# lich0031/AIDE

Measured on AMD Instinct MI355X. Metric: training images/sec FuseUNet 256x256x2 bs=4/GPU, higher is better.
Workload: dtype f32; 1 GPU; c2 fuseunet fwd+loss+bwd+Adam(amsgrad), 256x256 2-modal, bs=4/GPU, fp32; global_batch=4, parallelism=dp1

## Files before the change

aide_amd/csrc/conv3x3_winograd.hip:

```cpp
#include "common.h"

namespace {

struct WinoArgs {
    const float* x;
    const float* u;
    const float* bias;
    float* y;
    long x_bs, y_bs, split_stride;
    int N, Cin, H, W, Cout;
    int tiles_w, tiles_h, n_co_tiles, splitk, chunks_total, accumulate;
};

constexpr int WCK = 8;
constexpr int WTCO = 64;
constexpr int RROWS = 18, RRS = 24;
constexpr int RCS = RROWS * RRS + 8;
constexpr int RAWL = WCK * RCS;
constexpr int VL = 16 * 64 * WCK;
constexpr int UL = 16 * WTCO * WCK;
constexpr int WBUF = RAWL + VL + UL;

__global__ __launch_bounds__(256, 1) void conv3x3_wino_kernel(const WinoArgs a) {
    extern __shared__ __attribute__((aligned(16))) float lds[];
    const int tid = threadIdx.x, lane = tid & 63, wid = tid >> 6;
    const int half = lane >> 5, j = lane & 31;
    const int wave_m = wid >> 1, wave_n = wid & 1;

    int b = xcd_remap(blockIdx.x, gridDim.x);
    const int co_tile = b % a.n_co_tiles; b /= a.n_co_tiles;
    const int split = b % a.splitk;       b /= a.splitk;
    const int tw = b % a.tiles_w;         b /= a.tiles_w;
    const int th = b % a.tiles_h;
    const int n = b / a.tiles_h;
    const int h0 = th * 16, w0 = tw * 16, co0 = co_tile * WTCO;
    const int HW = a.H * a.W;

    const int cps = (a.chunks_total + a.splitk - 1) / a.splitk;
    const int c_begin = split * cps;
    const int c_end = min(c_begin + cps, a.chunks_total);

    constexpr int NRB = 3, NRC = 2, NU = UL / 4 / 256;
    unsigned offB[NRB], ldsB[NRB], offC[NRC], ldsC[NRC], offU[NU];
#pragma unroll
    for (int e = 0; e < NRB; ++e) {
        int q = tid + e * 256;
        if (q >= WCK * RROWS * 4) q -= 256;
        const int c = q / (RROWS * 4), rem = q - c * (RROWS * 4), r = rem / 4, s4 = rem - r * 4;
        const int ih = h0 - 1 + r, iw = w0 + 4 * s4;
        const bool ok = ih >= 0 && ih < a.H && iw < a.W;
        offB[e] = ok ? (unsigned)(c * HW + r * a.W + 1 + 4 * s4) * 4u : BUF_OOB;
        ldsB[e] = (unsigned)(c * RCS + r * RRS + 4 + 4 * s4);
    }
#pragma unroll
    for (int e = 0; e < NRC; ++e) {
        int q = tid + e * 256;
        if (q >= WCK * RROWS * 2) q -= 256;
        const int c = q / (RROWS * 2), rem = q - c * (RROWS * 2), r = rem / 2, side = rem - r * 2;
        const int ih = h0 - 1 + r, iw = side ? w0 + 16 : w0 - 1;
        const bool ok = ih >= 0 && ih < a.H && iw >= 0 && iw < a.W;
        offC[e] = ok ? (unsigned)(c * HW + r * a.W + (side ? 17 : 0)) * 4u : BUF_OOB;
        ldsC[e] = (unsigned)(c * RCS + r * RRS + (side ? 20 : 3));
    }
#pragma unroll
    for (int v = 0; v < NU; ++v) {
        const int f = tid + v * 256;
        const int pp = f / (WTCO * WCK / 4), w4 = f - pp * (WTCO * WCK / 4);
        offU[v] = (unsigned)(pp * a.Cout * WCK + w4 * 4) * 4u;
    }
    const __amdgpu_buffer_rsrc_t xrs =
        make_rsrc(a.x + (long)n * a.x_bs + (long)h0 * a.W + w0 - (a.W + 1));
    const __amdgpu_buffer_rsrc_t urs = make_rsrc(a.u + (long)co0 * WCK);

    f32x4 rb[NRB], ru[NU];
    float rc[NRC];
    auto fetch_raw = [&](int l, int chunk) {
        const unsigned xs = (unsigned)(min(chunk, c_end - 1) * WCK) * (unsigned)HW * 4u;
        if (l < NRB) rb[l] = buf_load_f32x4(xrs, offB[l], xs);
        else rc[l - NRB] = buf_load_f32(xrs, offC[l - NRB], xs);
    };
    auto put_raw = [&](int l, float* raw) {
        if (l < NRB) *reinterpret_cast<f32x4*>(raw + ldsB[l]) = rb[l];
        else raw[ldsC[l - NRB]] = rc[l - NRB];
    };
    auto fetch_u = [&](int v, int chunk) {
        const unsigned us = (unsigned)min(chunk, c_end - 1) * 16u * (unsigned)a.Cout * (unsigned)WCK * 4u;
        ru[v] = buf_load_f32x4(urs, offU[v], us);
    };
    auto put_u = [&](int v, float* ubuf) { *reinterpret_cast<f32x4*>(ubuf + (tid + v * 256) * 4) = ru[v]; };

    f32x2 td[16], to[16];
    const int xci = lane & 7, xtj = lane >> 3;
    const int xr_off = xci * RCS + 4 * wid * RRS + 3 + 2 * xtj;
    const int xw_off = (2 * wid * 8 + xtj) * WCK + xci;
    auto xf_read = [&](int i, const float* raw) {
        td[i].x = raw[xr_off + (i / 4) * RRS + (i % 4)];
        td[i].y = raw[xr_off + (2 + i / 4) * RRS + (i % 4)];
    };
    auto xf_math = [&]() {
        f32x2 tt[16];
#pragma unroll
        for (int c = 0; c < 4; ++c) {
            tt[c] = td[c] - td[8 + c]; tt[4 + c] = td[4 + c] + td[8 + c];
            tt[8 + c] = td[8 + c] - td[4 + c]; tt[12 + c] = td[4 + c] - td[12 + c];
        }
#pragma unroll
        for (int r = 0; r < 4; ++r) {
            to[r * 4] = tt[r * 4] - tt[r * 4 + 2]; to[r * 4 + 1] = tt[r * 4 + 1] + tt[r * 4 + 2];
            to[r * 4 + 2] = tt[r * 4 + 2] - tt[r * 4 + 1]; to[r * 4 + 3] = tt[r * 4 + 1] - tt[r * 4 + 3];
        }
    };
    auto xf_store = [&](int o, float* vbuf) {
        vbuf[o * 64 * WCK + xw_off] = to[o].x;
        vbuf[o * 64 * WCK + xw_off + 8 * WCK] = to[o].y;
    };

    f32x16 acc[16];
#pragma unroll
    for (int p = 0; p < 16; ++p)
#pragma unroll
        for (int r = 0; r < 16; ++r) acc[p][r] = 0.0f;

    float* set0 = lds;
    float* set1 = lds + WBUF;
#pragma unroll
    for (int l = 0; l < NRB + NRC; ++l) fetch_raw(l, c_begin);
#pragma unroll
    for (int v = 0; v < NU; ++v) fetch_u(v, c_begin);
#pragma unroll
    for (int l = 0; l < NRB + NRC; ++l) put_raw(l, set0);
#pragma unroll
    for (int v = 0; v < NU; ++v) put_u(v, set0 + RAWL + VL);
#pragma unroll
    for (int l = 0; l < NRB + NRC; ++l) fetch_raw(l, c_begin + 1);
    __syncthreads();
#pragma unroll
    for (int i = 0; i < 16; ++i) xf_read(i, set0);
    xf_math();
#pragma unroll
    for (int o = 0; o < 16; ++o) xf_store(o, set0 + RAWL);
#pragma unroll
    for (int l = 0; l < NRB + NRC; ++l) put_raw(l, set1);
    __syncthreads();

    int cur = 0;
    for (int chunk = c_begin; chunk < c_end; ++chunk) {
        float* sc = cur ? set1 : set0;
        float* sn = cur ? set0 : set1;
        const float* la = sc + RAWL + VL + (wave_m * 32 + j) * WCK + half * 4;
        const float* lb = sc + RAWL + (wave_n * 32 + j) * WCK + half * 4;
        constexpr int STEPS = 16 * (WCK / 2);
        f32x4 a0A, b0A, a1A, b1A, a0B, b0B, a1B, b1B;
        auto frag = [&](int p, f32x4& af, f32x4& bf) {
            af = *reinterpret_cast<const f32x4*>(la + p * WTCO * WCK);
            bf = *reinterpret_cast<const f32x4*>(lb + p * 64 * WCK);
        };
        auto slot = [&](int st, const f32x4& a0c, const f32x4& b0c, const f32x4& a1c, const f32x4& b1c,
                        f32x4& a0n, f32x4& b0n, f32x4& a1n, f32x4& b1n) {
            const int g2 = st >> 3, k = st & 7, q = k >> 1;
            if (k == 0 && g2 + 1 < 8) { frag(2 * g2 + 2, a0n, b0n); frag(2 * g2 + 3, a1n, b1n); }
            if (k & 1) acc[2 * g2 + 1] = __builtin_amdgcn_mfma_f32_32x32x2f32(a1c[q], b1c[q], acc[2 * g2 + 1], 0, 0, 0);
            else acc[2 * g2] = __builtin_amdgcn_mfma_f32_32x32x2f32(a0c[q], b0c[q], acc[2 * g2], 0, 0, 0);
            if (st < NU) fetch_u(st, chunk + 1);
            else if (st < NU + NRB + NRC) fetch_raw(st - NU, chunk + 2);
            if (st >= 4 && st < 20) xf_read(st - 4, sn);
            if (st == 24) xf_math();
            if (st >= 26 && st < 42) xf_store(st - 26, sn + RAWL);
            if (st >= 44 && st < 44 + NU) put_u(st - 44, sn + RAWL + VL);
            if (st >= 52 && st < 52 + NRB + NRC) put_raw(st - 52, sc);
            __builtin_amdgcn_sched_barrier(0);
        };
        frag(0, a0A, b0A); frag(1, a1A, b1A);
#pragma unroll
        for (int st = 0; st < STEPS; st += 16) {
#pragma unroll
            for (int k = 0; k < 8; ++k) slot(st + k, a0A, b0A, a1A, b1A, a0B, b0B, a1B, b1B);
#pragma unroll
            for (int k = 0; k < 8; ++k) slot(st + 8 + k, a0B, b0B, a1B, b1B, a0A, b0A, a1A, b1A);
        }
        __syncthreads();
        cur ^= 1;
    }

    float* yn = a.y + (long)split * a.split_stride + (long)n * a.y_bs;
    const bool add_bias = (a.bias != nullptr) && (split == 0);
    const int tile = wave_n * 32 + j, ti = tile >> 3, tj = tile & 7;
    const int oh = h0 + 2 * ti, ow = w0 + 2 * tj;
    const bool pok = oh < a.H && ow < a.W;
    float bvs[16];
#pragma unroll
    for (int r = 0; r < 16; ++r) {
        const int co = co0 + wave_m * 32 + (r & 3) + 8 * (r >> 2) + 4 * half;
        bvs[r] = (add_bias && pok && co < a.Cout) ? a.bias[co] : 0.f;
    }
#pragma unroll
    for (int r4 = 0; r4 < 16; r4 += 4) {
        float2 olds[4][2];
#pragma unroll
        for (int q = 0; q < 4; ++q) {
            const int co = co0 + wave_m * 32 + q + 8 * (r4 >> 2) + 4 * half;
#pragma unroll
            for (int i = 0; i < 2; ++i)
                olds[q][i] = (a.accumulate && pok && co < a.Cout)
                                 ? *reinterpret_cast<const float2*>(yn + (long)co * HW + (long)(oh + i) * a.W + ow) : make_float2(0.f, 0.f);
        }
#pragma unroll
        for (int q = 0; q < 4; ++q) {
            const int r = r4 + q;
            const int co = co0 + wave_m * 32 + (r & 3) + 8 * (r >> 2) + 4 * half;
            float s[2][4];
#pragma unroll
            for (int c = 0; c < 4; ++c) {
                const float m0 = acc[c][r], m1 = acc[4 + c][r], m2 = acc[8 + c][r], m3 = acc[12 + c][r];
                s[0][c] = m0 + m1 + m2;
                s[1][c] = m1 - m2 - m3;
            }
            if (pok && co < a.Cout) {
                const float bv = bvs[r];
#pragma unroll
                for (int i = 0; i < 2; ++i) {
                    float2 o;
                    o.x = s[i][0] + s[i][1] + s[i][2] + bv;
                    o.y = s[i][1] - s[i][2] - s[i][3] + bv;
                    float2* p = reinterpret_cast<float2*>(yn + (long)co * HW + (long)(oh + i) * a.W + ow);
                    o.x += olds[q][i].x; o.y += olds[q][i].y;
                    *p = o;
                }
            }
        }
    }
}

__global__ void wino_splitk_reduce_kernel(const float* __restrict__ slabs, long split_stride, int splitk,
                                          float* __restrict__ y, long y_bs, int C, int HW,
                                          const float* __restrict__ bias, int accumulate, long total) {
    for (long i = (long)blockIdx.x * blockDim.x + threadIdx.x; i < total;
         i += (long)gridDim.x * blockDim.x) {
        const long chw = (long)C * HW;
        const long n = i / chw, rem = i - n * chw;
        float v = slabs[i];
        for (int s = 1; s < splitk; ++s) v += slabs[(long)s * split_stride + i];
        if (bias) v += bias[rem / HW];
        float* p = y + n * y_bs + rem;
        if (accumulate) v += *p;
        *p = v;
    }
}
__global__ __launch_bounds__(256) void wino_splitk_reduce4_kernel(const float* __restrict__ slabs, long split_stride, int splitk,
                                                                  float* __restrict__ y, long y_bs, int C, int HW,
                                                                  const float* __restrict__ bias, int accumulate, long total4) {
    const long i = (long)blockIdx.x * blockDim.x + threadIdx.x;
    if (i >= total4) return;
    const long chw4 = (long)C * HW / 4;
    const long n = i / chw4, rem = (i - n * chw4) * 4;
    const float* sp = slabs + i * 4;
    f32x4 v = *reinterpret_cast<const f32x4*>(sp);
    int s = 1;
    for (; s + 4 <= splitk; s += 4) {
        const f32x4 t0 = *reinterpret_cast<const f32x4*>(sp + (long)s * split_stride);
        const f32x4 t1 = *reinterpret_cast<const f32x4*>(sp + (long)(s + 1) * split_stride);
        const f32x4 t2 = *reinterpret_cast<const f32x4*>(sp + (long)(s + 2) * split_stride);
        const f32x4 t3 = *reinterpret_cast<const f32x4*>(sp + (long)(s + 3) * split_stride);
        v = (((v + t0) + t1) + t2) + t3;
    }
    for (; s < splitk; ++s) v += *reinterpret_cast<const f32x4*>(sp + (long)s * split_stride);
    if (bias) v += bias[rem / HW];
    float* p = y + n * y_bs + rem;
    if (accumulate) v += *reinterpret_cast<const f32x4*>(p);
    *reinterpret_cast<f32x4*>(p) = v;
}

struct WinoPackDesc {
    const float* w; float* uf; float* ud;
    int Co, Ci, ci_pad, co_pad;
    long block_start;
};

__device__ __forceinline__ void wino_g(const float g[9], float u[16]) {
    float t[12];
#pragma unroll
    for (int c = 0; c < 3; ++c) {
        const float g0 = g[c], g1 = g[3 + c], g2 = g[6 + c];
        t[c] = g0; t[3 + c] = 0.5f * (g0 + g1 + g2); t[6 + c] = 0.5f * (g0 - g1 + g2); t[9 + c] = g2;
    }
#pragma unroll
    for (int r = 0; r < 4; ++r) {
        const float a0 = t[r * 3], a1 = t[r * 3 + 1], a2 = t[r * 3 + 2];
        u[r * 4] = a0; u[r * 4 + 1] = 0.5f * (a0 + a1 + a2); u[r * 4 + 2] = 0.5f * (a0 - a1 + a2); u[r * 4 + 3] = a2;
    }
}

constexpr int WP_T = 32;
__global__ __launch_bounds__(256) void wino_pack_multi_kernel(const WinoPackDesc* __restrict__ descs, int n) {
    __shared__ __attribute__((aligned(16))) float ot[16 * 256];
    const long blk = blockIdx.x;
    int lo = 0, hi = n - 1;
    while (lo < hi) {
        const int mid = (lo + hi + 1) >> 1;
        if (descs[mid].block_start <= blk) lo = mid; else hi = mid - 1;
    }
    const WinoPackDesc d = descs[lo];
    const int tid = threadIdx.x;
    const int tiles_ci = (d.Ci + WP_T - 1) / WP_T;
    const int tb = (int)(blk - d.block_start);
    const int co0 = (tb / tiles_ci) * WP_T, ci0 = (tb % tiles_ci) * WP_T;
    const int nci = min(WP_T, d.Ci - ci0);
    float g[9], u[16];
    const int lo3 = tid & 7, hi5 = tid >> 3;
    for (int grp = 0; grp < 8; ++grp) {
        const bool fwd = grp < 4;
        const int q = grp & 3;
        float* dst = fwd ? d.uf : d.ud;
        if (dst == nullptr) continue;
        const int co = fwd ? hi5 : 8 * q + lo3, ci = fwd ? 8 * q + lo3 : hi5;
        const bool live = fwd ? (ci0 + 8 * q < d.ci_pad) : (co0 + 8 * q < d.co_pad);
        if (!live) continue;
        {
            const bool in = co0 + co < d.Co && ci < nci;
            const float* wp = d.w + ((long)(co0 + co) * d.Ci + ci0 + ci) * 9;
#pragma unroll
            for (int t = 0; t < 9; ++t) g[t] = in ? wp[fwd ? t : 8 - t] : 0.f;
        }
        wino_g(g, u);
#pragma unroll
        for (int p = 0; p < 16; ++p) ot[p * 256 + tid] = u[p];
        __syncthreads();
        const int C = fwd ? d.Co : d.Ci, c0 = fwd ? co0 : ci0;
        const long gbase = (long)((fwd ? ci0 : co0) / 8 + q) * 16;
        const int nrun = min(WP_T, C - c0) * 8;
#pragma unroll
        for (int k = 0; k < 4; ++k) {
            const int f = tid + k * 256, p = f >> 6, x4 = (f & 63) * 4;
            if (x4 < nrun)
                *reinterpret_cast<f32x4*>(dst + ((gbase + p) * C + c0) * 8 + x4) =
                    *reinterpret_cast<const f32x4*>(ot + p * 256 + x4);
        }
        __syncthreads();
    }
}

}

extern "C" {

int aide_conv3x3_wino_supported(int Cin, int H, int W, int Cout) {
    return (H % 2 == 0 && W % 4 == 0 && Cout % 64 == 0 && Cin % 8 == 0) ? 1 : 0;
}

int aide_conv3x3_wino_splitk(int N, int Cin, int H, int W, int Cout) {
    const long nb = (long)((H + 15) / 16) * ((W + 15) / 16) * N * (Cout / 64);
    const int chunks = Cin / 8;
    int s = 1;
    while (nb * s < 200 && s * 2 <= chunks / 4) s *= 2;
    return s;
}

int aide_conv3x3_wino_pack_blocks(int Co, int Ci) {
    return ((Co + WP_T - 1) / WP_T) * ((Ci + WP_T - 1) / WP_T);
}

int aide_conv3x3_wino_pack_multi(const void* descs, int n, int64_t total_blocks, hipStream_t stream) {
    if (!descs || n <= 0 || total_blocks <= 0) return AIDE_ERR_ARG;
    static_assert(sizeof(WinoPackDesc) == 48, "descriptor layout");
    AIDE_LAUNCH_TIMED(AIDE_KT_OTHER, 0.0, wino_pack_multi_kernel, dim3((unsigned)total_blocks), dim3(256), 0, stream,
                       (const WinoPackDesc*)descs, n);
    return aide_launch_status();
}

int aide_conv3x3_wino(const float* x, int64_t x_bs, const float* u, const float* bias, float* y,
                      int64_t y_bs, int N, int Cin, int H, int W, int Cout, int accumulate, int splitk,
                      float* ws, hipStream_t stream) {
    if (!x || !u || !y || !aide_conv3x3_wino_supported(Cin, H, W, Cout) || x_bs % 4 || y_bs % 2)
        return AIDE_ERR_ARG;
    static AideLdsOptIn lds_opt;
    if (int rc = lds_opt.ensure([] {
            return hipFuncSetAttribute((const void*)conv3x3_wino_kernel, hipFuncAttributeMaxDynamicSharedMemorySize,
                                       2 * WBUF * (int)sizeof(float));
        })) return rc;
    WinoArgs a;
    a.x = x; a.u = u; a.x_bs = x_bs; a.N = N; a.Cin = Cin; a.H = H; a.W = W; a.Cout = Cout;
    a.tiles_w = (W + 15) / 16; a.tiles_h = (H + 15) / 16; a.n_co_tiles = Cout / WTCO;
    a.chunks_total = Cin / WCK;
    if (splitk < 1) splitk = 1;
    if (splitk > a.chunks_total) splitk = a.chunks_total;
    if (splitk > 1 && !ws) return AIDE_ERR_ARG;
    a.splitk = splitk;
    if (splitk > 1) {
        a.y = ws; a.y_bs = (long)Cout * H * W; a.split_stride = (long)N * Cout * H * W;
        a.bias = nullptr; a.accumulate = 0;
    } else {
        a.y = y; a.y_bs = y_bs; a.split_stride = 0; a.bias = bias; a.accumulate = (accumulate == 1);
    }
    const long nb = (long)a.tiles_w * a.tiles_h * N * a.n_co_tiles * splitk;
    AIDE_LAUNCH_TIMED(AIDE_KT_WINO2, AIDE_CONV_FLOPS(N, H, W, Cout, Cin), conv3x3_wino_kernel, dim3((unsigned)nb), dim3(256),
                      2 * WBUF * sizeof(float), stream, a);
    int rc = aide_launch_status();
    if (rc != 0) return rc;
    if (splitk > 1 && accumulate != 2) {
        const long total = (long)N * Cout * H * W;
        if ((H * W) % 4 == 0 && y_bs % 4 == 0) {
            AIDE_LAUNCH_TIMED(AIDE_KT_REDUCE, 0.0, wino_splitk_reduce4_kernel, dim3((unsigned)((total / 4 + 255) / 256)), dim3(256), 0, stream, ws,
                               total, splitk, y, (long)y_bs, Cout, H * W, bias, accumulate, total / 4);
        } else {
            const int blocks = (int)min((total + 255) / 256, (long)2048);
            AIDE_LAUNCH_TIMED(AIDE_KT_REDUCE, 0.0, wino_splitk_reduce_kernel, dim3(blocks), dim3(256), 0, stream, ws,
                               total, splitk, y, (long)y_bs, Cout, H * W, bias, accumulate, total);
        }
        rc = aide_launch_status();
    }
    return rc;
}

}
```

Measured before the change: 644.0 images/sec.

## Tune Winograd conv kernel: fast-div indexing, LDS swizzle, peeled first chunk, buffer-store epilogue

Replaces the runtime integer divisions in block-index decoding with precomputed magic-number division. Swizzles the LDS layout of the U and V tiles to cut bank conflicts on MFMA fragment reads and transform stores. Peels the first chunk so accumulators are seeded with zero inside the MFMA instead of being zeroed explicitly. The epilogue is rewritten to use buffer loads and stores with out-of-bounds masking, packed f32x2 math and hoisted old-value loads. It also handles empty split-k ranges through a zero-record descriptor. These changes add complexity and risk subtle indexing bugs, for example bias reads are no longer guarded by bounds.

```diff
diff --git a/aide_amd/csrc/conv3x3_winograd.hip b/aide_amd/csrc/conv3x3_winograd.hip
--- a/aide_amd/csrc/conv3x3_winograd.hip
+++ b/aide_amd/csrc/conv3x3_winograd.hip
@@ -1,6 +1,12 @@
 #include "common.h"
 
 namespace {
+
+struct FastDiv {
+    unsigned m;
+    int l, d;
+};
+__device__ __forceinline__ int fdiv(int n, FastDiv f) { return (int)((__umulhi((unsigned)n, f.m) + (unsigned)n) >> f.l); }
 
 struct WinoArgs {
     const float* x;
@@ -9,7 +15,8 @@
     float* y;
     long x_bs, y_bs, split_stride;
     int N, Cin, H, W, Cout;
-    int tiles_w, tiles_h, n_co_tiles, splitk, chunks_total, accumulate;
+    int chunks_total, chunks_per_split, accumulate;
+    FastDiv co_tiles, splitk, tiles_w, tiles_h;
 };
 
 constexpr int WCK = 8;
@@ -23,22 +30,22 @@
 
 __global__ __launch_bounds__(256, 1) void conv3x3_wino_kernel(const WinoArgs a) {
     extern __shared__ __attribute__((aligned(16))) float lds[];
-    const int tid = threadIdx.x, lane = tid & 63, wid = tid >> 6;
+    const int tid = threadIdx.x, lane = tid & 63, wid = __builtin_amdgcn_readfirstlane(tid >> 6);
     const int half = lane >> 5, j = lane & 31;
     const int wave_m = wid >> 1, wave_n = wid & 1;
 
-    int b = xcd_remap(blockIdx.x, gridDim.x);
-    const int co_tile = b % a.n_co_tiles; b /= a.n_co_tiles;
-    const int split = b % a.splitk;       b /= a.splitk;
-    const int tw = b % a.tiles_w;         b /= a.tiles_w;
-    const int th = b % a.tiles_h;
-    const int n = b / a.tiles_h;
+    int b = xcd_remap(blockIdx.x, gridDim.x), bq;
+    bq = fdiv(b, a.co_tiles); const int co_tile = b - bq * a.co_tiles.d; b = bq;
+    bq = fdiv(b, a.splitk);   const int split = b - bq * a.splitk.d;     b = bq;
+    bq = fdiv(b, a.tiles_w);  const int tw = b - bq * a.tiles_w.d;       b = bq;
+    const int n = fdiv(b, a.tiles_h), th = b - n * a.tiles_h.d;
     const int h0 = th * 16, w0 = tw * 16, co0 = co_tile * WTCO;
     const int HW = a.H * a.W;
 
-    const int cps = (a.chunks_total + a.splitk - 1) / a.splitk;
-    const int c_begin = split * cps;
-    const int c_end = min(c_begin + cps, a.chunks_total);
+    const int c_begin = split * a.chunks_per_split;
+    const bool empty = c_begin >= a.chunks_total;
+    const int c_end = empty ? c_begin + 1 : min(c_begin + a.chunks_per_split, a.chunks_total);
+    const unsigned nrec = empty ? 0u : BUF_OOB;
 
     constexpr int NRB = 3, NRC = 2, NU = UL / 4 / 256;
     unsigned offB[NRB], ldsB[NRB], offC[NRC], ldsC[NRC], offU[NU];
@@ -68,9 +75,10 @@
         const int pp = f / (WTCO * WCK / 4), w4 = f - pp * (WTCO * WCK / 4);
         offU[v] = (unsigned)(pp * a.Cout * WCK + w4 * 4) * 4u;
     }
-    const __amdgpu_buffer_rsrc_t xrs =
-        make_rsrc(a.x + (long)n * a.x_bs + (long)h0 * a.W + w0 - (a.W + 1));
-    const __amdgpu_buffer_rsrc_t urs = make_rsrc(a.u + (long)co0 * WCK);
+    const __amdgpu_buffer_rsrc_t xrs = __builtin_amdgcn_make_buffer_rsrc(
+        const_cast<float*>(a.x + (long)n * a.x_bs + (long)h0 * a.W + w0 - (a.W + 1)), 0, nrec, 0x00020000);
+    const __amdgpu_buffer_rsrc_t urs =
+        __builtin_amdgcn_make_buffer_rsrc(const_cast<float*>(a.u + (long)co0 * WCK), 0, nrec, 0x00020000);
 
     f32x4 rb[NRB], ru[NU];
     float rc[NRC];
@@ -87,12 +95,14 @@
         const unsigned us = (unsigned)min(chunk, c_end - 1) * 16u * (unsigned)a.Cout * (unsigned)WCK * 4u;
         ru[v] = buf_load_f32x4(urs, offU[v], us);
     };
-    auto put_u = [&](int v, float* ubuf) { *reinterpret_cast<f32x4*>(ubuf + (tid + v * 256) * 4) = ru[v]; };
+    const int uswz = tid ^ ((tid >> 4) & 1);
+    auto put_u = [&](int v, float* ubuf) { *reinterpret_cast<f32x4*>(ubuf + (uswz + v * 256) * 4) = ru[v]; };
 
     f32x2 td[16], to[16];
     const int xci = lane & 7, xtj = lane >> 3;
     const int xr_off = xci * RCS + 4 * wid * RRS + 3 + 2 * xtj;
     const int xw_off = (2 * wid * 8 + xtj) * WCK + xci;
+    const int xw_off1 = (2 * wid * 8 + 8 + xtj) * WCK + (xci ^ 4);
     auto xf_read = [&](int i, const float* raw) {
         td[i].x = raw[xr_off + (i / 4) * RRS + (i % 4)];
         td[i].y = raw[xr_off + (2 + i / 4) * RRS + (i % 4)];
@@ -112,14 +122,10 @@
     };
     auto xf_store = [&](int o, float* vbuf) {
         vbuf[o * 64 * WCK + xw_off] = to[o].x;
-        vbuf[o * 64 * WCK + xw_off + 8 * WCK] = to[o].y;
+        vbuf[o * 64 * WCK + xw_off1] = to[o].y;
     };
 
     f32x16 acc[16];
-#pragma unroll
-    for (int p = 0; p < 16; ++p)
-#pragma unroll
-        for (int r = 0; r < 16; ++r) acc[p][r] = 0.0f;
 
     float* set0 = lds;
     float* set1 = lds + WBUF;
@@ -143,24 +149,26 @@
     for (int l = 0; l < NRB + NRC; ++l) put_raw(l, set1);
     __syncthreads();
 
-    int cur = 0;
-    for (int chunk = c_begin; chunk < c_end; ++chunk) {
-        float* sc = cur ? set1 : set0;
-        float* sn = cur ? set0 : set1;
-        const float* la = sc + RAWL + VL + (wave_m * 32 + j) * WCK + half * 4;
-        const float* lb = sc + RAWL + (wave_n * 32 + j) * WCK + half * 4;
+    const int fhalf = (half ^ ((j >> 3) & 1)) * 4;
+    auto run_chunk = [&](int chunk, float* sc, float* sn, auto first) {
+        constexpr bool FIRST = decltype(first)::value;
+        const float* la = sc + RAWL + VL + (wave_m * 32 + j) * WCK + fhalf;
+        const float* lb = sc + RAWL + (wave_n * 32 + j) * WCK + fhalf;
         constexpr int STEPS = 16 * (WCK / 2);
         f32x4 a0A, b0A, a1A, b1A, a0B, b0B, a1B, b1B;
         auto frag = [&](int p, f32x4& af, f32x4& bf) {
             af = *reinterpret_cast<const f32x4*>(la + p * WTCO * WCK);
             bf = *reinterpret_cast<const f32x4*>(lb + p * 64 * WCK);
         };
+        auto mfma = [&](int p, int q, const f32x4& af, const f32x4& bf) {
+            acc[p] = __builtin_amdgcn_mfma_f32_32x32x2f32(af[q], bf[q], (FIRST && q == 0) ? f32x16{} : acc[p], 0, 0, 0);
+        };
         auto slot = [&](int st, const f32x4& a0c, const f32x4& b0c, const f32x4& a1c, const f32x4& b1c,
                         f32x4& a0n, f32x4& b0n, f32x4& a1n, f32x4& b1n) {
             const int g2 = st >> 3, k = st & 7, q = k >> 1;
             if (k == 0 && g2 + 1 < 8) { frag(2 * g2 + 2, a0n, b0n); frag(2 * g2 + 3, a1n, b1n); }
-            if (k & 1) acc[2 * g2 + 1] = __builtin_amdgcn_mfma_f32_32x32x2f32(a1c[q], b1c[q], acc[2 * g2 + 1], 0, 0, 0);
-            else acc[2 * g2] = __builtin_amdgcn_mfma_f32_32x32x2f32(a0c[q], b0c[q], acc[2 * g2], 0, 0, 0);
+            if (k & 1) mfma(2 * g2 + 1, q, a1c, b1c);
+            else mfma(2 * g2, q, a0c, b0c);
             if (st < NU) fetch_u(st, chunk + 1);
             else if (st < NU + NRB + NRC) fetch_raw(st - NU, chunk + 2);
             if (st >= 4 && st < 20) xf_read(st - 4, sn);
@@ -179,54 +187,72 @@
             for (int k = 0; k < 8; ++k) slot(st + 8 + k, a0B, b0B, a1B, b1B, a0A, b0A, a1A, b1A);
         }
         __syncthreads();
+    };
+    run_chunk(c_begin, set0, set1, std::true_type{});
+    int cur = 1;
+    for (int chunk = c_begin + 1; chunk < c_end; ++chunk) {
+        run_chunk(chunk, cur ? set1 : set0, cur ? set0 : set1, std::false_type{});
         cur ^= 1;
     }
 
-    float* yn = a.y + (long)split * a.split_stride + (long)n * a.y_bs;
-    const bool add_bias = (a.bias != nullptr) && (split == 0);
     const int tile = wave_n * 32 + j, ti = tile >> 3, tj = tile & 7;
     const int oh = h0 + 2 * ti, ow = w0 + 2 * tj;
     const bool pok = oh < a.H && ow < a.W;
-    float bvs[16];
-#pragma unroll
-    for (int r = 0; r < 16; ++r) {
-        const int co = co0 + wave_m * 32 + (r & 3) + 8 * (r >> 2) + 4 * half;
-        bvs[r] = (add_bias && pok && co < a.Cout) ? a.bias[co] : 0.f;
-    }
-#pragma unroll
-    for (int r4 = 0; r4 < 16; r4 += 4) {
-        float2 olds[4][2];
-#pragma unroll
-        for (int q = 0; q < 4; ++q) {
-            const int co = co0 + wave_m * 32 + q + 8 * (r4 >> 2) + 4 * half;
+    const int cw = co0 + wave_m * 32;
+    float* const yw = a.y + (long)split * a.split_stride + (long)n * a.y_bs + (long)cw * HW;
+    const __amdgpu_buffer_rsrc_t yrs = make_rsrc(yw);
+    const unsigned yoff = pok ? (unsigned)(4 * half * HW + oh * a.W + ow) * 4u : BUF_OOB;
+    auto ysoff = [&](int r, int i, int x) {
+        return (unsigned)(((r & 3) + 8 * (r >> 2)) * HW + i * a.W + x) * 4u;
+    };
+    f32x2 bvs[8];
+    const bool add_bias = (a.bias != nullptr) && (split == 0);
+    const float* bw = a.bias + cw + 4 * half;
+#pragma unroll
+    for (int rp = 0; rp < 8; ++rp) {
+        const int r = 2 * rp, co = (r & 3) + 8 * (r >> 2);
+        bvs[rp] = add_bias ? f32x2{bw[co], bw[co + 1]} : f32x2{0.f, 0.f};
+    }
+    auto sub = [](f32x2 x, f32x2 y) {
+        f32x2 r;
+        asm("v_pk_add_f32 %0, %1, %2 neg_lo:[0,1] neg_hi:[0,1]" : "=v"(r) : "v"(x), "v"(y));
+        return r;
+    };
+    {
+        const __amdgpu_buffer_rsrc_t ors = __builtin_amdgcn_make_buffer_rsrc(yw, 0, a.accumulate ? BUF_OOB : 0u, 0x00020000);
+        f32x2 olds[8][2][2];
+#pragma unroll
+        for (int rp = 0; rp < 8; ++rp)
 #pragma unroll
             for (int i = 0; i < 2; ++i)
-                olds[q][i] = (a.accumulate && pok && co < a.Cout)
-                                 ? *reinterpret_cast<const float2*>(yn + (long)co * HW + (long)(oh + i) * a.W + ow) : make_float2(0.f, 0.f);
-        }
-#pragma unroll
-        for (int q = 0; q < 4; ++q) {
-            const int r = r4 + q;
-            const int co = co0 + wave_m * 32 + (r & 3) + 8 * (r >> 2) + 4 * half;
-            float s[2][4];
+#pragma unroll
+                for (int x = 0; x < 2; ++x)
+                    olds[rp][i][x] = f32x2{buf_load_f32(ors, yoff, ysoff(2 * rp, i, x)), buf_load_f32(ors, yoff, ysoff(2 * rp + 1, i, x))};
+        __builtin_amdgcn_sched_barrier(0);
+#pragma unroll
+        for (int rp = 0; rp < 8; ++rp) {
+            const int r = 2 * rp;
+#pragma unroll
+            for (int p = 0; p < 16; ++p) asm volatile("" : "+a"(acc[p]));
+            f32x2 s[2][4];
 #pragma unroll
             for (int c = 0; c < 4; ++c) {
-                const float m0 = acc[c][r], m1 = acc[4 + c][r], m2 = acc[8 + c][r], m3 = acc[12 + c][r];
+                const f32x2 m0 = {acc[c][r], acc[c][r + 1]}, m1 = {acc[4 + c][r], acc[4 + c][r + 1]};
+                const f32x2 m2 = {acc[8 + c][r], acc[8 + c][r + 1]}, m3 = {acc[12 + c][r], acc[12 + c][r + 1]};
                 s[0][c] = m0 + m1 + m2;
-                s[1][c] = m1 - m2 - m3;
+                s[1][c] = sub(sub(m1, m2), m3);
             }
-            if (pok && co < a.Cout) {
-                const float bv = bvs[r];
-#pragma unroll
-                for (int i = 0; i < 2; ++i) {
-                    float2 o;
-                    o.x = s[i][0] + s[i][1] + s[i][2] + bv;
-                    o.y = s[i][1] - s[i][2] - s[i][3] + bv;
-                    float2* p = reinterpret_cast<float2*>(yn + (long)co * HW + (long)(oh + i) * a.W + ow);
-                    o.x += olds[q][i].x; o.y += olds[q][i].y;
-                    *p = o;
-                }
+#pragma unroll
+            for (int i = 0; i < 2; ++i) {
+                f32x2 ox = s[i][0] + s[i][1] + s[i][2] + bvs[rp];
+                f32x2 oy = sub(sub(s[i][1], s[i][2]), s[i][3]) + bvs[rp];
+                ox += olds[rp][i][0]; oy += olds[rp][i][1];
+                __builtin_amdgcn_raw_buffer_store_b32(__float_as_uint(ox.x), yrs, yoff, ysoff(r, i, 0), 0);
+                __builtin_amdgcn_raw_buffer_store_b32(__float_as_uint(oy.x), yrs, yoff, ysoff(r, i, 1), 0);
+                __builtin_amdgcn_raw_buffer_store_b32(__float_as_uint(ox.y), yrs, yoff, ysoff(r + 1, i, 0), 0);
+                __builtin_amdgcn_raw_buffer_store_b32(__float_as_uint(oy.y), yrs, yoff, ysoff(r + 1, i, 1), 0);
             }
+            __builtin_amdgcn_sched_barrier(0);
         }
     }
 }
@@ -339,6 +365,14 @@
     }
 }
 
+FastDiv fast_div(int d) {
+    FastDiv f;
+    f.d = d; f.l = 0;
+    while ((1L << f.l) < d) ++f.l;
+    f.m = (unsigned)((((1ULL << 32) * ((1ULL << f.l) - (unsigned long long)d)) / (unsigned long long)d) + 1);
+    return f;
+}
+
 }
 
 extern "C" {
@@ -379,19 +413,21 @@
         })) return rc;
     WinoArgs a;
     a.x = x; a.u = u; a.x_bs = x_bs; a.N = N; a.Cin = Cin; a.H = H; a.W = W; a.Cout = Cout;
-    a.tiles_w = (W + 15) / 16; a.tiles_h = (H + 15) / 16; a.n_co_tiles = Cout / WTCO;
+    const int tiles_w = (W + 15) / 16, tiles_h = (H + 15) / 16, co_tiles = Cout / WTCO;
     a.chunks_total = Cin / WCK;
     if (splitk < 1) splitk = 1;
     if (splitk > a.chunks_total) splitk = a.chunks_total;
     if (splitk > 1 && !ws) return AIDE_ERR_ARG;
-    a.splitk = splitk;
+    a.chunks_per_split = (a.chunks_total + splitk - 1) / splitk;
+    a.co_tiles = fast_div(co_tiles); a.splitk = fast_div(splitk); a.tiles_w = fast_div(tiles_w); a.tiles_h = fast_div(tiles_h);
     if (splitk > 1) {
         a.y = ws; a.y_bs = (long)Cout * H * W; a.split_stride = (long)N * Cout * H * W;
         a.bias = nullptr; a.accumulate = 0;
     } else {
         a.y = y; a.y_bs = y_bs; a.split_stride = 0; a.bias = bias; a.accumulate = (accumulate == 1);
     }
-    const long nb = (long)a.tiles_w * a.tiles_h * N * a.n_co_tiles * splitk;
+    const long nb = (long)tiles_w * tiles_h * N * co_tiles * splitk;
+    if (nb >= (1L << 31)) return AIDE_ERR_ARG;
     AIDE_LAUNCH_TIMED(AIDE_KT_WINO2, AIDE_CONV_FLOPS(N, H, W, Cout, Cin), conv3x3_wino_kernel, dim3((unsigned)nb), dim3(256),
                       2 * WBUF * sizeof(float), stream, a);
     int rc = aide_launch_status();
```

Result: no change. 643.1 images/sec, median of 3 (-0.1%).
